# unitaryai/VTC

Measured on AMD Instinct MI355X. Metric: video-text pairs encoded/sec (config 3: 8-frame TimeSformer video + title + 5 comments, CAM) + 10k x 10k sim+R@K ms, higher is better.
Workload: dtype bf16 (video tower) + f16 (text tower blocks), fp32 accumulate; 1 GPU; configs/pretrained_clip_timesformer_comments_attention.jsonc PretrainedCLIP_TimeSformer_finaltf forward: 1024 pairs/GPU/step = 1024 videos (8 x 3 x 224 x 224) + 1024 titles + 5120 comments (77 tokens) + CAM + sim; pairs_per_gpu=1024, frames=8, text_tower=ragged: tokens after EOT are not computed, identical outputs, parallelism=dp1 (one process per GPU, no collective in the encode path)

## Files before the change

### vtc_amd/csrc/gemm.hip

```cpp
#include "gemm_common.h"
#include "ln_row.h"

#if defined(VTC_ABLATE_STORES) || defined(VTC_ABLATE_DMA) || defined(VTC_ABLATE_HALF_DMA) || defined(VTC_ABLATE_DMA_EXEC1) || \
    defined(VTC_ABLATE_VMWAIT) || defined(VTC_ABLATE_LDSREAD) || defined(VTC_PROBE_MFMA32) || defined(VTC_PHASED_WAIT_FIRST) || \
    defined(VTC_PHASED_ONE_BARRIER) || defined(VTC_NO_RELAXED_FIRST) || defined(VTC_ROW_PANEL_PROBE)
#error "timing-probe macros are not part of the product source any more (see the note above)"
#endif
#include "gemm_stamps.h"

using namespace vtcgemm;

namespace {

constexpr int MFMA_PRIO = 3;
constexpr int SMALL_NSTAGE = 3;

template <int CTRL>
__device__ __forceinline__ float dpp_f(float x) {
  return __int_as_float(__builtin_amdgcn_update_dpp(0, __float_as_int(x), CTRL, 0xf, 0xf, false));
}

template <bool NT>
__device__ __forceinline__ void store16(void *o, uint4 v) {
  typedef unsigned v4u_t __attribute__((ext_vector_type(4)));
// ... 97 lines not shown
        unsigned bits;
        if constexpr (NPL != 4) bits = __float_as_uint(acc[i][j][e]);
        else bits = (unsigned)max(__float_as_int((rn - 2.0f * acc[i][j][e]) + cn[j][e]), 0);
        constexpr unsigned KMASK = NPL != 4 ? 0x8000007Fu : 127u;
        unsigned kr = key_bfi(KMASK, (unsigned)(16 * j + 4 * g + e), bits), kc = key_bfi(KMASK, (unsigned)(16 * i + l15), bits);
        if constexpr (!INTERIOR) {
          const bool v = mv && ((cvalid >> (4 * j + e)) & 1);
          kr = v ? kr : VTC_L2MIN_INF;
          kc = v ? kc : VTC_L2MIN_INF;
        }
        row.insert(kr);
        if (cols_too) col[j][e].insert(kc);
      }
  };
#pragma unroll
  for (int i = 0; i < TM; ++i) {
    const int m = mbase + 16 * i + l15;
    const bool mv = m < p.M;
    MinR row;
    row.init();
    if (interior) row_pass(i, std::true_type{}, row);
    else row_pass(i, std::false_type{}, row);
    {
      const bool odd = (g & 1) != 0, up = g >= 2;
      unsigned o[NPLR];
#pragma unroll
      for (int q = 0; q < NPLR; ++q) o[q] = xor16_of(row.v[q], odd);
      row.merge(o);
#pragma unroll
      for (int q = 0; q < NPLR; ++q) o[q] = xor32_of(row.v[q], up);
      row.merge(o);
    }
    if (mv && nbase < p.N && g < NPLR) {
      unsigned mine = row.v[0];
#pragma unroll
      for (int q = 1; q < NPLR; ++q) mine = g == q ? row.v[q] : mine;
      p.epi.rowk[(size_t)g * rstride + (size_t)cblk * p.M + m] = mine;
    }
  }
  if (cols_too) {
    const size_t cstride = (size_t)p.epi.nblk_r * p.N;
    const int rblk = mbase / (TM * 16);
#define VTC_DPPU(x, ctrl) (unsigned)__builtin_amdgcn_update_dpp(0, (int)(x), ctrl, 0xf, 0xf, false)
    auto xor4 = [](unsigned x) -> unsigned {
      int r = __builtin_amdgcn_update_dpp(0, (int)x, 0x104, 0xf, 0x5, false);
      r = __builtin_amdgcn_update_dpp(r, (int)x, 0x114, 0xf, 0xA, false);
      return (unsigned)r;
    };
    auto step = [&](const Min4 &lo, const Min4 &hi, bool up, auto fetch) __attribute__((always_inline)) -> Min4 {
      Min4 k;
      unsigned got[NPL];
#pragma unroll
      for (int q = 0; q < NPL; ++q) {
        k.v[q] = up ? hi.v[q] : lo.v[q];
        got[q] = fetch(up ? lo.v[q] : hi.v[q]);
      }
      k.merge(got);
      return k;
    };
    const bool b0 = (l15 & 1) != 0, b1 = (l15 & 2) != 0, b2 = (l15 & 4) != 0, b3 = (l15 & 8) != 0;
    Min4 s8[8], s4[4], s2[2];
#pragma unroll
    for (int c = 0; c < 8; ++c)
      s8[c] = step(col[c >> 2][c & 3], col[(c + 8) >> 2][c & 3], b0, [](unsigned x) { return VTC_DPPU(x, 0xB1); });
#pragma unroll
    for (int c = 0; c < 4; ++c) s4[c] = step(s8[c], s8[c + 4], b1, [](unsigned x) { return VTC_DPPU(x, 0x4E); });
#pragma unroll
    for (int c = 0; c < 2; ++c) s2[c] = step(s4[c], s4[c + 2], b3, [](unsigned x) { return VTC_DPPU(x, 0x128); });
    const Min4 fin = step(s2[0], s2[1], b2, xor4);
#undef VTC_DPPU
    const int cj = (b0 ? 2 : 0) + (b1 ? 1 : 0), ce = (b3 ? 2 : 0) + (b2 ? 1 : 0);
    const int n = nbase + 16 * cj + 4 * g + ce;
    if (n < p.N && mbase < p.M) {
      unsigned *dst = p.epi.colk + (size_t)rblk * p.N + n;
#pragma unroll
      for (int q = 0; q < NPL; ++q) dst[q * cstride] = fin.v[q];
    }
  }
}

template <typename OutT, int TM>
constexpr int fast_epilogue_trailing_stores() { return TM * (sizeof(OutT) == 2 ? 2 : 4); }

template <typename T, int MODE_T, typename OutT, int WM, int WN, int TM, int TN, int SCRATCH_PER_WAVE, bool REJOIN = false>
__device__ __forceinline__ void tile_epilogue(f32x4 (&acc)[TM][TN], const GemmParams &p, int m0, int n0, unsigned scratch_off) {
  constexpr bool FOLD = MODE_T >= EPI_FOLD_BASE && MODE_T <= EPI_RESID_FOLD_C;
  constexpr bool CENTER = MODE_T == EPI_RESID_FOLD_C;
  constexpr int MODE = CENTER ? VTC_EPI_RESID : (FOLD ? MODE_T - EPI_FOLD_BASE : MODE_T);
  auto rejoin = [&]() __attribute__((always_inline)) {
    if constexpr (REJOIN) {
      if ((int)(threadIdx.x >> 6) / WN == 0) __builtin_amdgcn_s_barrier();
    }
  };
  if constexpr (MODE == EPI_L2MIN || l2min_half_keys(MODE)) {
    rejoin();
    if constexpr (TN == 4) l2min_epilogue<WM, WN, TM, TN, l2min_row_planes(MODE), l2min_col_planes(MODE)>(acc, p, m0, n0);
    return;
  }
  extern __shared__ __attribute__((aligned(16))) char lds[];
  constexpr int BM = WM * TM * 16, BN = WN * TN * 16;
  int tid = threadIdx.x;
  asm volatile("" : "+v"(tid));
  const int lane = tid & 63, wave = tid >> 6;
  const int wr = wave / WN, wc = wave % WN;
  const int g = lane >> 4;
  const int ldo = p.ldo;
  const bool vec_ok = (ldo & 3) == 0;
  constexpr bool nt_out = MODE == EPI_L2DIST || (sizeof(OutT) == 2 && MODE != VTC_EPI_RESID && MODE != EPI_RESID_LN);
  const bool interior = (m0 + BM <= p.M) && (n0 + BN <= p.N) && vec_ok;
  float scale = 1.0f;
  if (MODE == EPI_SCALE) scale = __expf(*p.epi.scale_log);
  if constexpr (sizeof(OutT) == 2) {
    if (interior) {
      constexpr int TSB = 136;
      char *trb = lds + scratch_off + wave * SCRATCH_PER_WAVE;
      const int l15 = lane & 15;
      const int ncol0 = n0 + wc * TN * 16;
      float4 b4[TN];
      if (p.bias) {
#pragma unroll
        for (int j = 0; j < TN; ++j) b4[j] = *reinterpret_cast<const float4 *>(p.bias + ncol0 + 16 * j + 4 * g);
      } else {
#pragma unroll
        for (int j = 0; j < TN; ++j) b4[j] = make_float4(0.f, 0.f, 0.f, 0.f);
      }
      [[maybe_unused]] float *fold_rs = reinterpret_cast<float *>(trb + 2 * 16 * TSB);
      [[maybe_unused]] float *fold_sc = fold_rs + 2 * TM * 16;
      constexpr int NQ = (TM * 16 + 63) / 64;
      [[maybe_unused]] float2 fst[NQ];
      [[maybe_unused]] float4 fsc = make_float4(0.f, 0.f, 0.f, 0.f);
      if constexpr (FOLD) {
        static_assert(2 * 16 * TSB + (2 * TM * 16 + TN * 16) * 4 <= SCRATCH_PER_WAVE, "folded LayerNorm: row statistics + s in the wave's scratch");
#pragma unroll
        for (int q = 0; q < NQ; ++q) {
          const int r = min(lane + 64 * q, TM * 16 - 1);
          fst[q] = *reinterpret_cast<const float2 *>(p.epi.fold_stat + 2 * (size_t)(m0 + wr * TM * 16 + r));
        }
        fsc = *reinterpret_cast<const float4 *>(p.epi.fold_s + ncol0 + 4 * (lane & (TN * 4 - 1)));
      }
      rejoin();
      if constexpr (FOLD) {
#pragma unroll
        for (int q = 0; q < NQ; ++q) {
          const int r = lane + 64 * q;
          if (TM * 16 % 64 == 0 || r < TM * 16) *reinterpret_cast<float2 *>(fold_rs + 2 * r) = fst[q];
        }
        if (lane < TN * 4) *reinterpret_cast<float4 *>(fold_sc + 4 * lane) = fsc;
        __builtin_amdgcn_fence(__ATOMIC_RELEASE, "wavefront");
        __builtin_amdgcn_wave_barrier();
        __builtin_amdgcn_fence(__ATOMIC_ACQUIRE, "wavefront");
      }
      auto put = [&](int i) __attribute__((always_inline)) {
        char *buf = trb + (i & 1) * (16 * TSB);
#pragma unroll
        for (int j = 0; j < TN; ++j) {
          float v0, v1, v2, v3;
          if constexpr (FOLD) {
            const float2 st = *reinterpret_cast<const float2 *>(fold_rs + 2 * (i * 16 + l15));
            const float4 sj = *reinterpret_cast<const float4 *>(fold_sc + 16 * j + 4 * g);
            typedef float f2_t __attribute__((ext_vector_type(2)));
            const f2_t nmu = {-st.x, -st.x}, rs = {st.y, st.y};
            const f2_t t01 = __builtin_elementwise_fma(nmu, (f2_t){sj.x, sj.y}, (f2_t){acc[i][j][0], acc[i][j][1]});
            const f2_t t23 = __builtin_elementwise_fma(nmu, (f2_t){sj.z, sj.w}, (f2_t){acc[i][j][2], acc[i][j][3]});
            const f2_t w01 = __builtin_elementwise_fma(rs, t01, (f2_t){b4[j].x, b4[j].y});
            const f2_t w23 = __builtin_elementwise_fma(rs, t23, (f2_t){b4[j].z, b4[j].w});
            v0 = w01.x; v1 = w01.y; v2 = w23.x; v3 = w23.y;
          } else {
            v0 = acc[i][j][0] + b4[j].x; v1 = acc[i][j][1] + b4[j].y; v2 = acc[i][j][2] + b4[j].z; v3 = acc[i][j][3] + b4[j].w;
          }
          if (MODE == VTC_EPI_GELU) {
            if constexpr (sizeof(T) == 4) {
              v0 = quick_gelu<true>(v0); v1 = quick_gelu<true>(v1); v2 = quick_gelu<true>(v2); v3 = quick_gelu<true>(v3);
            } else {
              const gelu_f2_t g01 = quick_gelu2((gelu_f2_t){v0, v1}), g23 = quick_gelu2((gelu_f2_t){v2, v3});
              v0 = g01.x; v1 = g01.y; v2 = g23.x; v3 = g23.y;
            }
          }
          uint2 pk;
          pk.x = pack16<OutT>(v0, v1);
          pk.y = pack16<OutT>(v2, v3);
          *reinterpret_cast<uint2 *>(buf + l15 * TSB + j * 32 + g * 8) = pk;
        }
      };
      static_assert(2 * 16 * TSB <= SCRATCH_PER_WAVE, "two transposition buffers per wave");
      static_assert(fast_epilogue_trailing_stores<OutT, TM>() == TM * 2, "16-bit fast path: TM fragment rows x 2 stores (the loop below)");
      char *out_base16;
      {
        const int m0s = __builtin_amdgcn_readfirstlane(m0), wrs = __builtin_amdgcn_readfirstlane(wr), ncs = __builtin_amdgcn_readfirstlane(ncol0);
        out_base16 = reinterpret_cast<char *>(reinterpret_cast<unsigned short *>(p.out) + (size_t)(m0s + wrs * TM * 16) * ldo + ncs);
      }
      put(0);
#pragma unroll
      for (int i = 0; i < TM; ++i) {
        __builtin_amdgcn_fence(__ATOMIC_RELEASE, "wavefront");
        __builtin_amdgcn_wave_barrier();
        __builtin_amdgcn_fence(__ATOMIC_ACQUIRE, "wavefront");
        const char *buf = trb + (i & 1) * (16 * TSB);
        uint2 lo[2], hi[2];
#pragma unroll
        for (int k = 0; k < 2; ++k) {
          const int r = (lane >> 3) + 8 * k, c = lane & 7;
          lo[k] = *reinterpret_cast<const uint2 *>(buf + r * TSB + c * 16);
          hi[k] = *reinterpret_cast<const uint2 *>(buf + r * TSB + c * 16 + 8);
        }
        if (i + 1 < TM) put(i + 1);
#pragma unroll
        for (int k = 0; k < 2; ++k) {
          char *o = out_base16 + (unsigned)(((i * 16 + (lane >> 3) + 8 * k) * ldo + (lane & 7) * 8) * 2);
          store16<nt_out>(o, make_uint4(lo[k].x, lo[k].y, hi[k].x, hi[k].y));
        }
      }
      __builtin_amdgcn_fence(__ATOMIC_RELEASE, "wavefront");
      __builtin_amdgcn_wave_barrier();
      return;
    }
  }
  [[maybe_unused]] __amdgpu_buffer_rsrc_t out_rsrc;
  [[maybe_unused]] const int m0u = __builtin_amdgcn_readfirstlane(m0);
  if constexpr (MODE == EPI_RESID_LN || MODE == VTC_EPI_RESID) {
    const size_t rem = (size_t)(p.M - m0u) * ldo * 4;
    out_rsrc = __builtin_amdgcn_make_buffer_rsrc(reinterpret_cast<float *>(p.out) + (size_t)m0u * ldo, 0,
                                                 (int)(rem < 0xFFFFFFF0u ? rem : 0xFFFFFFF0u), 0x00020000);
  }
  if (sizeof(OutT) == 4 && interior) {
    constexpr int TS = 68;
    constexpr int H = TN / 4, NP = TM * H;
    static_assert(TN % 4 == 0 && (H == 1 || sizeof(OutT) == 4), "wide wave tiles: fp32 outputs only");
    static_assert(sizeof(OutT) == 2 || fast_epilogue_trailing_stores<OutT, TM>() <= NP * 4, "fp32 fast path: NP passes x 4 stores (>= the count the K loop's relaxed waits assume)");
    float *tr = reinterpret_cast<float *>(lds + scratch_off + wave * SCRATCH_PER_WAVE);
    const int l15 = lane & 15;
    const int ncol0 = n0 + wc * TN * 16;
    const float *colv = MODE == EPI_L2DIST ? p.epi.coln : p.bias;
    float cadd[H][8];
#pragma unroll
    for (int hh = 0; hh < H; ++hh)
#pragma unroll
      for (int e = 0; e < 8; ++e) cadd[hh][e] = 0.f;
    if (colv) {
#pragma unroll
      for (int hh = 0; hh < H; ++hh) {
        const float4 c4 = *reinterpret_cast<const float4 *>(colv + ncol0 + 64 * hh + l15 * 4);
        cadd[hh][0] = c4.x; cadd[hh][1] = c4.y; cadd[hh][2] = c4.z; cadd[hh][3] = c4.w;
      }
    }
    auto fin = [&](float a, float add) -> float {
      float v = a + add;
      if (MODE == VTC_EPI_GELU) v = quick_gelu<sizeof(T) == 4>(v);
      if (MODE == EPI_SCALE) v *= scale;
      return v;
    };
    auto x_ptr = [&](int pp, int k) -> float * {
      const int m = m0 + (wr * TM + pp / H) * 16 + (lane >> 4) + 4 * k;
      return reinterpret_cast<float *>(p.out) + (size_t)m * ldo + ncol0 + 64 * (pp % H) + l15 * 4;
    };
    constexpr int XD = 2;
    float4 xr[XD][4];
    constexpr bool SPLIT = FOLD && MODE == VTC_EPI_RESID && sizeof(T) == 2;
    [[maybe_unused]] float *mean_prev = tr + 16 * TS;
    [[maybe_unused]] float2 *stat_buf = reinterpret_cast<float2 *>(tr + 16 * TS + TM * 16);
    constexpr int NQM = (TM * 16 + 63) / 64;
    [[maybe_unused]] float mprev[NQM];
    if constexpr (SPLIT && CENTER) {
      static_assert((16 * TS + TM * 16) * 4 <= SCRATCH_PER_WAVE, "folded LayerNorm: previous means in the wave's scratch");
#pragma unroll
      for (int q = 0; q < NQM; ++q) mprev[q] = p.epi.fold_stat[2 * (size_t)(m0 + wr * TM * 16 + min(lane + 64 * q, TM * 16 - 1))];
    }
    typedef unsigned v2u_t __attribute__((ext_vector_type(2)));
    [[maybe_unused]] char *hi_base = nullptr, *lo_base = nullptr;
    [[maybe_unused]] unsigned split_off0 = 0, split_row4 = 0;
    if constexpr (SPLIT) {
      const int m0s = __builtin_amdgcn_readfirstlane(m0);
      const int wrs = __builtin_amdgcn_readfirstlane(wr), ncs = __builtin_amdgcn_readfirstlane(ncol0);
      const size_t row0 = (size_t)(m0s + wrs * TM * 16) * ldo + ncs;
      hi_base = reinterpret_cast<char *>(reinterpret_cast<unsigned short *>(p.epi.y16) + row0);
      lo_base = reinterpret_cast<char *>(reinterpret_cast<unsigned short *>(p.epi.y16lo) + row0);
      split_off0 = (unsigned)(((lane >> 4) * ldo + l15 * 4) * 2);
      split_row4 = (unsigned)ldo * 8u;
    }
    auto split_off = [&](int pp, int k) -> unsigned { return split_off0 + (unsigned)(4 * (pp / H) + k) * split_row4 + (unsigned)(128 * (pp % H)); };
    auto x_load = [&](int pp, int k) -> float4 {
      if constexpr (SPLIT) {
        const v2u_t hi = *reinterpret_cast<const v2u_t *>(hi_base + split_off(pp, k));
        const v2u_t lo = *reinterpret_cast<const v2u_t *>(lo_base + split_off(pp, k));
        return make_float4(__uint_as_float(hi.x), __uint_as_float(hi.y), __uint_as_float(lo.x), __uint_as_float(lo.y));
      } else {
        return *reinterpret_cast<const float4 *>(x_ptr(pp, k));
      }
    };
    [[maybe_unused]] unsigned skip_rem = 1, skip_step = 0, skip_m = 0;
    if constexpr (MODE == VTC_EPI_RESID || MODE == EPI_RESID_LN) {
      if (p.epi.skip_mod > 0) {
        skip_m = (unsigned)p.epi.skip_mod;
// ... 265 lines not shown
      const unsigned w_addr = lds_base + cur * STAGE + A_BYTES + wrow;
#pragma unroll
      for (int ks = 0; ks < 2; ++ks) {
        if (ks == 1 && late_dma) issued = stage_ahead(t, NSTAGE - 1);
        const unsigned coff = ((4 * ks + g) ^ swz) << 4;
        u32x4 wf[TN], aE, aO;
#pragma unroll
        for (int j = 0; j < TN; ++j) lds_read16(wf[j], w_addr + coff, j * 16 * ROWB);
        lds_read16(aE, a_addr + coff, 0);
#pragma unroll
        for (int i = 0; i < TM; i += 2) {
          lds_read16(aO, a_addr + coff, (i + 1) * 16 * ROWB);
          if (i == 0) lgkm_wait_frags<1>(aE, wf);
          else lgkm_wait<1>(aE);
#pragma unroll
          for (int j = 0; j < TN; ++j) Mma<T>::run(wf[j], aE, acc[i][j]);
          if (i + 2 < TM) {
            lds_read16(aE, a_addr + coff, (i + 2) * 16 * ROWB);
            lgkm_wait<1>(aO);
          } else {
            lgkm_wait<0>(aO);
          }
#pragma unroll
          for (int j = 0; j < TN; ++j) Mma<T>::run(wf[j], aO, acc[i + 1][j]);
        }
      }
      if (issued) ++ahead;
      wait_all_but(ahead - 1);
      --ahead;
      __syncthreads();
      cur = cur + 1 == NSTAGE ? 0 : cur + 1;
    }

    tile_epilogue<T, MODE, OutT, WM, WN, TM, TN, STAGE / NW>(acc, p, m0, n0, ((cur + NSTAGE - 1) % NSTAGE) * STAGE);
    if (has_next) __syncthreads();

    if (!has_next) break;
    li += nb_x; m0 = m0n; n0 = n0n;
    tile_offsets<AG>(a_off, m0, p.M, p.lda_bytes, wave_u, lane);
    tile_offsets<WG>(w_off, n0, p.N, p.ldw_bytes, wave_u, lane);
    has_next = li + nb_x < nt_x;
    if (has_next) decode(start_x + li + nb_x, m0n, n0n);
  }
}


template <typename T16>
__device__ __attribute__((noinline)) void fused_ln_rows(const float *out, int M, int N, int m0, const float *ln_g, const float *ln_b,
                                                        T16 *ln_out) {
  typedef unsigned v4u_t __attribute__((ext_vector_type(4)));
  const __amdgpu_buffer_rsrc_t x_rsrc = __builtin_amdgcn_make_buffer_rsrc(const_cast<float *>(out), 0, (int)((size_t)M * N * 4), 0x00020000);
  const int lane = threadIdx.x & 63, wave = threadIdx.x >> 6;
  const int width = N;
  const int rows = min(256, M - m0);
  constexpr int RB = 8;
  for (int r0 = wave; r0 < rows; r0 += 8 * RB) {
    float4 v[RB][LN_MAXV][2];
#pragma unroll
    for (int b = 0; b < RB; ++b) {
      const int r = min(r0 + 8 * b, rows - 1);
#pragma unroll
      for (int i = 0; i < LN_MAXV; ++i) {
        const int c = min((lane + 64 * i) * 8, width - 8);
        const int off = (int)(((size_t)(m0 + r) * width + c) * 4);
        const v4u_t a = __builtin_amdgcn_raw_buffer_load_b128(x_rsrc, off, 0, 16);
        const v4u_t b4 = __builtin_amdgcn_raw_buffer_load_b128(x_rsrc, off + 16, 0, 16);
        v[b][i][0] = make_float4(__uint_as_float(a.x), __uint_as_float(a.y), __uint_as_float(a.z), __uint_as_float(a.w));
        v[b][i][1] = make_float4(__uint_as_float(b4.x), __uint_as_float(b4.y), __uint_as_float(b4.z), __uint_as_float(b4.w));
      }
    }
#pragma unroll
    for (int b = 0; b < RB; ++b) {
      const int r = r0 + 8 * b;
      if (r < rows) ln_row_compute<T16, false>(v[b], ln_g, ln_b, ln_out + (size_t)(m0 + r) * width, width, lane);
    }
  }
}

template <int MODE, typename OutT, typename T, int DEEP = 0>
__global__ __launch_bounds__(512, 2) void gemm_phased_kernel(GemmParams p) {
  static_assert(sizeof(T) == 2, "16-bit operands (bf16 or IEEE half)");
  static_assert(DEEP == 0 || DEEP == 1, "0 = one quarter in flight, 1 = deep (W0 re-read)");
  constexpr int WM = 2, WN = 4, TM = 8, TN = 4, NW = 8, BM = 256, BN = 256;
  if (p.epi.m_dev) {
    p.M = *p.epi.m_dev;
    p.MT = (p.M + BM - 1) / BM;
  }
  constexpr int A_BYTES = BM * ROWB, STAGE = (BM + BN) * ROWB;
  extern __shared__ __attribute__((aligned(16))) char lds[];
  const int tid = threadIdx.x, lane = tid & 63, wave = tid >> 6;
  const int wr = wave >> 2, wc = wave & 3;
  const int g = lane >> 4;

  [[maybe_unused]] const int bid = blockIdx.x;
  const XcdRange rng = xcd_range(p.MT * p.NT);
  const int nb_x = rng.nb_x, nt_x = rng.nt_x, start_x = rng.start_x;
  auto decode = [&](int logical, int &m0, int &n0) { decode_tile<BM, BN>(logical, 1, p.MT, p.NT, m0, n0); };
  int li = rng.slot;
  if (li >= nt_x) return;
  int m0, n0;
  decode(start_x + li, m0, n0);
  int m0n = 0, n0n = 0;
  bool has_next = li + nb_x < nt_x;
  if (has_next) decode(start_x + li + nb_x, m0n, n0n);

  const int ksteps = p.K / 64;
  const unsigned lds_base = __builtin_amdgcn_readfirstlane((unsigned)(size_t)(lds_void *)lds);
  const int wave_u = __builtin_amdgcn_readfirstlane(wave);
  const int swz = (lane >> 1) & 7;
  const unsigned a_rd = (wr * 128 + (lane & 15)) * ROWB;
  const unsigned w_rd = A_BYTES + (wc * 64 + (lane & 15)) * ROWB;
  const unsigned coff0 = ((0 + g) ^ swz) << 4, coff1 = ((4 + g) ^ swz) << 4;
  unsigned ra0 = lds_base + a_rd + coff0, ra1 = lds_base + a_rd + coff1, rw0 = lds_base + w_rd + coff0, rw1 = lds_base + w_rd + coff1;
  int rd_step = STAGE;

  const int ga0 = (wave_u >> 2) * 16 + (wave_u & 3) * 2;
  const int gw0 = (wave_u >> 1) * 8 + (wave_u & 1) * 2;
  const unsigned a_vo = (unsigned)(lane >> 3) * (unsigned)p.lda_bytes + (((lane & 7) ^ (lane >> 4)) << 4);
  const unsigned w_vo = (unsigned)(lane >> 3) * (unsigned)p.ldw_bytes + (((lane & 7) ^ (lane >> 4)) << 4);
  const unsigned a_vo2 = (a_vo ^ 64u) + 8u * (unsigned)p.lda_bytes - 1024u, w_vo2 = (w_vo ^ 64u) + 8u * (unsigned)p.ldw_bytes - 1024u;
  const unsigned offA0 = (unsigned)ga0 * 8u * (unsigned)p.lda_bytes, offA1 = (unsigned)(ga0 + 8) * 8u * (unsigned)p.lda_bytes;
  const unsigned offW0 = (unsigned)gw0 * 8u * (unsigned)p.ldw_bytes, offW1 = (unsigned)(gw0 + 4) * 8u * (unsigned)p.ldw_bytes;
  const char *tbA = p.A + (size_t)m0 * p.lda_bytes, *tbW = p.W + (size_t)n0 * p.ldw_bytes;
  const char *tbAn = p.A + (size_t)m0n * p.lda_bytes, *tbWn = p.W + (size_t)n0n * p.ldw_bytes;
  auto stage2 = [&](const char *base, const char *tile_base, unsigned grp_off, int row0, int nrows, int ld_bytes, unsigned vo, unsigned vo2, int grp,
                    int kb, unsigned lds_dst, bool fast) __attribute__((always_inline)) {
    if (__builtin_expect(fast, 1)) {
      const char *sb0 = tile_base + (grp_off + (unsigned)kb);
      asm volatile(
          "s_mov_b32 m0, %3\n\t"
          "s_nop 0\n\t"
          "global_load_lds_dwordx4 %0, %2\n\t"
          "global_load_lds_dwordx4 %1, %2 offset:1024"
          :
          : "v"(vo), "v"(vo2), "s"(sb0), "s"(lds_dst)
          : "memory");
    } else {
#pragma unroll
      for (int q = 0; q < 2; ++q) {
        const int r = (grp + q) * 8 + (lane >> 3);
        const int c = (lane & 7) ^ ((r >> 1) & 7);
        int gr = row0 + r;
        gr = gr < nrows ? gr : nrows - 1;
        glds16(base + (size_t)gr * ld_bytes + kb + c * 16, __builtin_amdgcn_readfirstlane(lds_dst + q * 1024));
      }
    }
  };
  constexpr bool CAN_GATHER = MODE == EPI_PATCH && sizeof(T) == 2;
  const bool gather = CAN_GATHER && p.epi.gather;
  [[maybe_unused]] unsigned gvo[4] = {0, 0, 0, 0};
  [[maybe_unused]] const int g_cs = p.epi.patch == 32 ? 2 : 1;
  auto gather_offsets = [&](int sm) __attribute__((always_inline)) {
    if constexpr (CAN_GATHER) {
      const int P = p.epi.P, G = p.epi.grid, res = p.epi.res, ps = p.epi.patch;
#pragma unroll
      for (int h = 0; h < 2; ++h)
#pragma unroll
        for (int q = 0; q < 2; ++q) {
          const int m = min(sm + (ga0 + 8 * h + q) * 8 + (lane >> 3), p.M - 1);
          const int f = m / P, np = m - f * P;
          const int gy = np / G, gx = np - gy * G;
          const int c = ((lane & 7) ^ (lane >> 4)) ^ (q << 2);
          const unsigned origin = (unsigned)(((f * 3) * res + gy * ps) * res + gx * ps) * 2u;
          gvo[2 * h + q] = origin + (unsigned)((c >> g_cs) * res * 2 + ((c & ((1 << g_cs) - 1)) << 4));
        }
    }
  };
  auto gather_kbase = [&](int kk) -> size_t {
    const int k = kk * 64, pp = p.epi.patch * p.epi.patch;
    const int c = k / pp, i = (k - c * pp) / p.epi.patch;
    return ((size_t)c * p.epi.res + i) * p.epi.res * 2;
  };
  enum { Q_A0 = 0, Q_W0 = 1, Q_W1 = 2, Q_A1 = 3 };
  auto stage_quarter = [&](int qi, int sm, int sn, int kk, unsigned st, bool fastA, bool fastW, const char *ta, const char *tw) __attribute__((always_inline)) {
    if (qi == Q_A0 || qi == Q_A1) {
      const int grp = ga0 + (qi == Q_A1 ? 8 : 0);
      if constexpr (CAN_GATHER) {
        if (gather) {
          const char *sb0 = reinterpret_cast<const char *>(p.A) + gather_kbase(kk);
          const char *sb1 = sb0 - 1024;
          const int h = qi == Q_A1 ? 1 : 0;
          asm volatile(
              "s_mov_b32 m0, %4\n\t"
              "s_nop 0\n\t"
              "global_load_lds_dwordx4 %0, %2\n\t"
              "global_load_lds_dwordx4 %1, %3 offset:1024"
              :
              : "v"(gvo[2 * h]), "v"(gvo[2 * h + 1]), "s"(sb0), "s"(sb1), "s"(st + grp * 1024)
              : "memory");
          return;
        }
      }
      stage2(p.A, ta, qi == Q_A1 ? offA1 : offA0, sm, p.M, p.lda_bytes, a_vo, a_vo2, grp, kk * ROWB, st + grp * 1024, fastA);
    } else {
      const int grp = gw0 + (qi == Q_W1 ? 4 : 0);
      stage2(p.W, tw, qi == Q_W1 ? offW1 : offW0, sn, p.N, p.ldw_bytes, w_vo, w_vo2, grp, kk * ROWB, st + A_BYTES + grp * 1024, fastW);
    }
  };

  int cur = 0;
  {
    const bool fa = m0 + BM <= p.M, fw = n0 + BN <= p.N;
    if (gather) gather_offsets(m0);
#pragma unroll
    for (int qi = 0; qi < 4; ++qi) stage_quarter(qi, m0, n0, 0, lds_base, fa, fw, tbA, tbW);
    asm volatile("s_waitcnt vmcnt(0)" ::: "memory");
    __builtin_amdgcn_s_barrier();
  }

  u32x4 aS[4][2], wS[2][2];
  bool relax_first = false;
  [[maybe_unused]] float *nrm = reinterpret_cast<float *>(lds + 2 * STAGE);
  [[maybe_unused]] auto fetch_norm = [&](int tm0, int tn0) -> float {
    if (tid < 256) {
      const int m = tm0 + tid;
      return m < p.M ? -0.5f * p.epi.rown[m] : 0.f;
    }
    const int n = tn0 + tid - 256;
    return n < p.N ? -0.5f * p.epi.coln[n] : 0.f;
  };
  if constexpr (l2min_half_keys(MODE)) {
    nrm[tid] = fetch_norm(m0, n0);
    __syncthreads();
  }
  VTC_STAMP_INIT();
  while (true) {
    if (wr == 1) __builtin_amdgcn_s_barrier();
    f32x4 acc[TM][TN];
#pragma unroll
    for (int i = 0; i < TM; ++i)
#pragma unroll
      for (int j = 0; j < TN; ++j) {
        if constexpr (l2min_half_keys(MODE)) {
          const float hr = nrm[wr * 128 + 16 * i + (lane & 15)];
          const float4 hc = *reinterpret_cast<const float4 *>(nrm + 256 + wc * 64 + 16 * j + 4 * g);
          acc[i][j] = (f32x4){hr + hc.x, hr + hc.y, hr + hc.z, hr + hc.w};
        } else {
          acc[i][j] = (f32x4){0.f, 0.f, 0.f, 0.f};
        }
      }

    auto kloop = [&](auto all_fast_c) __attribute__((always_inline)) {
    constexpr bool ALL_FAST = decltype(all_fast_c)::value;
    for (int t = 0; t < ksteps; ++t) {
      const unsigned st_cur = lds_base + cur * STAGE, st_nxt = lds_base + (cur ^ 1) * STAGE;
      if constexpr (DEEP == 0) {
        const int kn = t + 1;
        const bool to_next = kn == ksteps && has_next;
        const int sm = to_next ? m0n : m0, sn = to_next ? n0n : n0, kk = kn < ksteps ? kn : 0;
        const bool fastA = ALL_FAST || sm + BM <= p.M, fastW = ALL_FAST || sn + BN <= p.N;
        const char *ta = to_next ? tbAn : tbA, *tw = to_next ? tbWn : tbW;
        if constexpr (CAN_GATHER) {
          if (gather && to_next) gather_offsets(m0n);
        }
        static_for<4>([&](auto ph_c) __attribute__((always_inline)) {
          constexpr int ph = decltype(ph_c)::value;
          constexpr int qm = ph >> 1, qn = (ph == 1 || ph == 2) ? 1 : 0;
          if constexpr (ph != 2) {
  #pragma unroll
            for (int j = 0; j < 2; ++j) {
              lds_read16(wS[j][0], rw0, (qn * 2 + j) * 16 * ROWB);
              lds_read16(wS[j][1], rw1, (qn * 2 + j) * 16 * ROWB);
            }
          }
          if constexpr (ph == 0 || ph == 2) {
  #pragma unroll
            for (int i = 0; i < 4; ++i) {
              lds_read16(aS[i][0], ra0, (qm * 4 + i) * 16 * ROWB);
              lds_read16(aS[i][1], ra1, (qm * 4 + i) * 16 * ROWB);
            }
          }
          stage_quarter(ph, sm, sn, kk, st_nxt, fastA, fastW, ta, tw);
          __builtin_amdgcn_s_barrier();
          lgkm_wait_subtile(aS, wS);
          __builtin_amdgcn_s_setprio(MFMA_PRIO);
  #pragma unroll
          for (int ks = 0; ks < 2; ++ks)
  #pragma unroll
            for (int i = 0; i < 4; ++i)
  #pragma unroll
              for (int j = 0; j < 2; ++j) Mma<T>::run(wS[j][ks], aS[i][ks], acc[qm * 4 + i][qn * 2 + j]);
          __builtin_amdgcn_s_setprio(0);
          constexpr int NST = fast_epilogue_trailing_stores<OutT, TM>();
          if (ph < 2 && t == 0 && relax_first) {
            if constexpr (ph == 0) asm volatile("s_waitcnt vmcnt(%0)" ::"n"(2 + NST) : "memory");
            else asm volatile("s_waitcnt vmcnt(%0)" ::"n"(4 + NST) : "memory");
          } else
            asm volatile("s_waitcnt vmcnt(2)" ::: "memory");
          __builtin_amdgcn_s_barrier();
        });
      } else {
        constexpr int NST = fast_epilogue_trailing_stores<OutT, TM>();
        const bool first = t == 0, last = t == ksteps - 1;
        const bool nx1 = t + 1 == ksteps && has_next;
        const int sm1 = nx1 ? m0n : m0, sn1 = nx1 ? n0n : n0, kk1 = t + 1 < ksteps ? t + 1 : 0;
        const bool fA1 = ALL_FAST || sm1 + BM <= p.M, fW1 = ALL_FAST || sn1 + BN <= p.N;
        const char *ta1 = nx1 ? tbAn : tbA, *tw1 = nx1 ? tbWn : tbW;
        const bool nx2 = t + 2 >= ksteps && has_next;
        const int sm2 = nx2 ? m0n : m0, sn2 = nx2 ? n0n : n0, kk2 = t + 2 < ksteps ? t + 2 : 0;
        const bool fA2 = ALL_FAST || sm2 + BM <= p.M, fW2 = ALL_FAST || sn2 + BN <= p.N;
        const char *ta2 = nx2 ? tbAn : tbA, *tw2 = nx2 ? tbWn : tbW;
        static_for<4>([&](auto ph_c) __attribute__((always_inline)) {
          constexpr int ph = decltype(ph_c)::value;
          constexpr int qm = ph >> 1, qn = (ph == 1 || ph == 2) ? 1 : 0;
          if constexpr (ph == 0 || ph == 1 || ph == 3) {
#pragma unroll
            for (int j = 0; j < 2; ++j) {
              lds_read16(wS[j][0], rw0, (qn * 2 + j) * 16 * ROWB);
              lds_read16(wS[j][1], rw1, (qn * 2 + j) * 16 * ROWB);
            }
          }
          if constexpr (ph == 0 || ph == 2) {
#pragma unroll
            for (int i = 0; i < 4; ++i) {
              lds_read16(aS[i][0], ra0, (qm * 4 + i) * 16 * ROWB);
              lds_read16(aS[i][1], ra1, (qm * 4 + i) * 16 * ROWB);
            }
          }
          if constexpr (ph == 0) {
            stage_quarter(Q_W0, sm1, sn1, kk1, st_nxt, fA1, fW1, ta1, tw1);
            if (first) stage_quarter(Q_A0, sm1, sn1, kk1, st_nxt, fA1, fW1, ta1, tw1);
          } else if constexpr (ph == 1) {
            if (first) stage_quarter(Q_W1, sm1, sn1, kk1, st_nxt, fA1, fW1, ta1, tw1);
            stage_quarter(Q_A1, sm1, sn1, kk1, st_nxt, fA1, fW1, ta1, tw1);
            if (first && relax_first) asm volatile("s_waitcnt vmcnt(%0)" ::"n"(8 + NST) : "memory");
            else asm volatile("s_waitcnt vmcnt(8)" ::: "memory");
          } else if constexpr (ph == 2) {
            if (!last) {
              if constexpr (CAN_GATHER) {
                if (gather && nx2 && t + 2 == ksteps) gather_offsets(m0n);
              }
              stage_quarter(Q_A0, sm2, sn2, kk2, st_cur, fA2, fW2, ta2, tw2);
            }
          } else {
            if (!last) stage_quarter(Q_W1, sm2, sn2, kk2, st_cur, fA2, fW2, ta2, tw2);
            lgkm_wait_w4(wS);
            if (last) asm volatile("s_waitcnt vmcnt(2)" ::: "memory");
            else asm volatile("s_waitcnt vmcnt(6)" ::: "memory");
          }
          __builtin_amdgcn_s_barrier();
          lgkm_wait_subtile(aS, wS);
          VTC_PHASE_STAMP(1);
          __builtin_amdgcn_s_setprio(MFMA_PRIO);
#pragma unroll
          for (int ks = 0; ks < 2; ++ks)
#pragma unroll
            for (int i = 0; i < 4; ++i)
#pragma unroll
              for (int j = 0; j < 2; ++j) Mma<T>::run(wS[j][ks], aS[i][ks], acc[qm * 4 + i][qn * 2 + j]);
          __builtin_amdgcn_s_setprio(0);
          VTC_PHASE_STAMP(0);
          __builtin_amdgcn_s_barrier();
        });
      }
      cur ^= 1;
      ra0 += rd_step; ra1 += rd_step; rw0 += rd_step; rw1 += rd_step;
      rd_step = -rd_step;
    }
    };
    if constexpr (MODE != EPI_L2MIN && !l2min_half_keys(MODE) && MODE != EPI_PATCH && MODE != EPI_RESID_LN) {
      const bool this_in = m0 + BM <= p.M && n0 + BN <= p.N, next_in = !has_next || (m0n + BM <= p.M && n0n + BN <= p.N);
      if (this_in && next_in) kloop(std::true_type{});
      else kloop(std::false_type{});
    } else {
      kloop(std::false_type{});
    }
    VTC_STAMP(0);
    VTC_STAMP(1);

    [[maybe_unused]] float nrm_next = 0.f;
    if constexpr (l2min_half_keys(MODE)) {
      if (has_next) nrm_next = fetch_norm(m0n, n0n);
    }
    tile_epilogue<T, MODE, OutT, WM, WN, TM, TN, STAGE / NW, true>(acc, p, m0, n0, (cur ^ 1) * STAGE);
    if constexpr (MODE == EPI_RESID_LN) {
      int *ticket = reinterpret_cast<int *>(lds + 2 * STAGE);
      asm volatile("s_waitcnt vmcnt(0)" ::: "memory");
      __syncthreads();
      if (tid == 0) *ticket = __hip_atomic_fetch_add(p.epi.ln_cnt + m0 / BM, 1, __ATOMIC_RELAXED, __HIP_MEMORY_SCOPE_AGENT);
      __syncthreads();
      if (*ticket == p.NT - 1)
        fused_ln_rows<T>(reinterpret_cast<const float *>(p.out), p.M, p.N, m0, p.epi.ln_g, p.epi.ln_b, reinterpret_cast<T *>(p.epi.ln_out));
    }
    VTC_STAMP_TILE_END(!has_next);
    if (!has_next) break;
    relax_first = MODE != EPI_L2MIN && !l2min_half_keys(MODE) && MODE != EPI_RESID_LN && (m0 + BM <= p.M) && (n0 + BN <= p.N) && ((p.ldo & 3) == 0);
    if constexpr (l2min_half_keys(MODE)) {
      nrm[tid] = nrm_next;
      asm volatile("s_waitcnt lgkmcnt(0)" ::: "memory");
    }
    __builtin_amdgcn_s_barrier();
    VTC_STAMP(3);
    li += nb_x; m0 = m0n; n0 = n0n;
    tbA = tbAn; tbW = tbWn;
    has_next = li + nb_x < nt_x;
    if (has_next) {
      decode(start_x + li + nb_x, m0n, n0n);
      tbAn = p.A + (size_t)m0n * p.lda_bytes; tbWn = p.W + (size_t)n0n * p.ldw_bytes;
    }
  }
}


}
namespace vtcgemm {
int num_cus() {
  static std::atomic<int> cus[64];
  int dev = 0;
  if (hipGetDevice(&dev) != hipSuccess || dev < 0 || dev >= 64) dev = 0;
  int n = cus[dev].load(std::memory_order_relaxed);
  if (n == 0) {
    int v = 0;
    if (hipDeviceGetAttribute(&v, hipDeviceAttributeMultiprocessorCount, dev) != hipSuccess || v <= 0) v = 256;
    cus[dev].store(n = v, std::memory_order_relaxed);
  }
  return n;
}
}
namespace {

template <typename T, int MODE, typename OutT, int WM, int WN, int TM, int TN, int NSTAGE>
int run(GemmParams p, hipStream_t stream) {
  constexpr int BM = WM * TM * 16, BN = WN * TN * 16, NT_ = WM * WN * 64;
  p.MT = cdiv(p.M, BM); p.NT = cdiv(p.N, BN);
  const int S = p.epi.ksplit > 1 ? p.epi.ksplit : 1;
  const int ntiles = p.MT * p.NT * S;
  const size_t shmem = (size_t)NSTAGE * (BM + BN) * ROWB;
  if (p.K / S / Mma<T>::KPR < NSTAGE - 1) { vtc_set_error("gemm: K=%d (/ %d slices) is too short for %d stages", p.K, S, NSTAGE); return 1; }
  const int wg_per_cu = shmem > 80 * 1024 ? 1 : 2;
  const int grid = min(ntiles, num_cus() * wg_per_cu);
  if (S > 1 && (grid < ntiles || p.K % (S * Mma<T>::KPR) != 0)) {
    vtc_set_error("gemm: split-K x %d needs one workgroup per (tile, slice) (%d > %d resident) and K %% (slices x %d) == 0 (K=%d)", S, ntiles, grid, Mma<T>::KPR, p.K);
    return 1;
  }
  static PerDeviceOnce attr;
  if (ensure_dynamic_lds(attr, reinterpret_cast<const void *>(&gemm_kernel<T, MODE, OutT, WM, WN, TM, TN, NSTAGE>), (int)shmem, "gemm")) return 1;
  hipLaunchKernelGGL((gemm_kernel<T, MODE, OutT, WM, WN, TM, TN, NSTAGE>), dim3(grid), dim3(NT_), shmem, stream, p);
  VTC_LAUNCH_CHECK("gemm");
  return 0;
}

template <int MODE, typename OutT, typename T, int DEEP>
int run_phased_d(GemmParams p, hipStream_t stream) {
  p.MT = cdiv(p.M, 256); p.NT = cdiv(p.N, 256);
  const int ntiles = p.MT * p.NT;
  const size_t shmem = (size_t)2 * 512 * ROWB + (MODE == EPI_RESID_LN ? 16 : 0) + (l2min_half_keys(MODE) ? 2048 : 0);
  const int grid = min(ntiles, num_cus());
  static PerDeviceOnce attr;
  if (ensure_dynamic_lds(attr, reinterpret_cast<const void *>(&gemm_phased_kernel<MODE, OutT, T, DEEP>), (int)shmem, "gemm_phased")) return 1;
  VTC_STAMP_HOST_BEFORE(p, stream);
  hipLaunchKernelGGL((gemm_phased_kernel<MODE, OutT, T, DEEP>), dim3(grid), dim3(512), shmem, stream, p);
  VTC_STAMP_HOST_AFTER(p, stream, grid, MODE);
  VTC_LAUNCH_CHECK("gemm_phased");
  return 0;
}
template <int MODE, typename OutT, typename T>
int run_phased(const GemmParams &p, hipStream_t stream) {
  if constexpr (MODE != EPI_RESID_LN && MODE != EPI_L2MIN && !l2min_half_keys(MODE)) {
    if (p.K >= 128) return run_phased_d<MODE, OutT, T, 1>(p, stream);
  }
  return run_phased_d<MODE, OutT, T, 0>(p, stream);
}

enum class Tile { Phased256, Small128, Small64 };
struct TileChoice {
  Tile tile;
  int nstage;
};
constexpr TileChoice choose_tile(int M, int N, int K, int elem_bytes, int ksplit, int cus) {
  const int ksteps = K / (ksplit > 1 ? ksplit : 1) / (ROWB / elem_bytes);
  const TileChoice small64 = {Tile::Small64, ksteps >= SMALL_NSTAGE - 1 ? SMALL_NSTAGE : 2};
  if (ksplit > 1) return small64;
  if (elem_bytes == 2) {
    const long tb = (long)cdiv(M, 256) * cdiv(N, 256), ts = (long)cdiv(M, 128) * cdiv(N, 128);
    const long rb = (tb + cus - 1) / cus, rs = (ts + 2 * cus - 1) / (2 * cus);
    if (rb * 100 <= rs * 65) return {Tile::Phased256, 2};
  }
  const long ts128 = (long)cdiv(M, 128) * cdiv(N, 128);
  if (ts128 * 2 <= cus) return small64;
  return {Tile::Small128, 2};
}
constexpr Tile tile_at_256_cus(int M, int N, int elem_bytes = 2) { return choose_tile(M, N, 768, elem_bytes, 0, 256).tile; }
static_assert(tile_at_256_cus(12800, 768) == Tile::Phased256, "150 big tiles: big");
static_assert(tile_at_256_cus(25344, 768) == Tile::Small128, "297 big tiles: small");
static_assert(tile_at_256_cus(6400, 768) == Tile::Small128, "75 big tiles: small");
static_assert(tile_at_256_cus(32768, 512) == Tile::Phased256, "256 big tiles: big");
static_assert(tile_at_256_cus(38400, 768) == Tile::Phased256, "450 big tiles: big");
static_assert(tile_at_256_cus(12800, 768, 4) != Tile::Phased256 && tile_at_256_cus(32768, 512, 4) != Tile::Phased256, "fp32 operands: never the phased kernel");
static_assert(tile_at_256_cus(1024, 2048) == Tile::Small64 && tile_at_256_cus(1024 + 128, 2048) == Tile::Small128, "64 x 64 while tiles128 * 2 <= cus");
static_assert(choose_tile(128, 128, 64, 2, 0, 256).nstage == 2 && choose_tile(128, 128, 128, 2, 0, 256).nstage == SMALL_NSTAGE &&
                  choose_tile(128, 128, 192, 2, 0, 256).nstage == SMALL_NSTAGE && choose_tile(128, 128, 256, 2, 4, 256).nstage == 2,
              "64 x 64 stages: 2 for one K-step (of a slice), 3 from two K-steps on");

template <typename T, int MODE, typename OutT>
int run_cfg(const GemmParams &p, hipStream_t stream) {
  const TileChoice c = choose_tile(p.M, p.N, p.K, sizeof(T), p.epi.ksplit, num_cus());
  if constexpr (sizeof(T) == 2) {
    if (c.tile == Tile::Phased256) return run_phased<MODE, OutT, T>(p, stream);
  }
  if (c.tile == Tile::Small64) {
    if (c.nstage == SMALL_NSTAGE) return run<T, MODE, OutT, 2, 1, 2, 4, SMALL_NSTAGE>(p, stream);
    return run<T, MODE, OutT, 2, 1, 2, 4, 2>(p, stream);
  }
  return run<T, MODE, OutT, 2, 2, 4, 4, 2>(p, stream);
}

int run_l2min(const GemmParams &p, hipStream_t stream) {
  if (p.epi.mode == EPI_L2MIN2) return run_phased<EPI_L2MIN2, float, bf16_t>(p, stream);
  if (p.epi.mode == EPI_L2MIN3) return run_phased<EPI_L2MIN3, float, bf16_t>(p, stream);
  return run_phased<EPI_L2MIN, float, bf16_t>(p, stream);
}

template <typename T>
int dispatch(GemmParams p, hipStream_t stream) {
  const bool out_f32 = p.epi.out_dtype == VTC_F32;
  using Out16 = std::conditional_t<sizeof(T) == 2, T, bf16_t>;
  switch (p.epi.mode) {
    case VTC_EPI_STORE:
      if (out_f32) return run_cfg<T, VTC_EPI_STORE, float>(p, stream);
      if constexpr (sizeof(T) == 2) {
        if (p.epi.fold_stat) return run_cfg<T, EPI_STORE_FOLD, Out16>(p, stream);
      }
      return run_cfg<T, VTC_EPI_STORE, Out16>(p, stream);
    case VTC_EPI_GELU:
      if (out_f32) return run_cfg<T, VTC_EPI_GELU, float>(p, stream);
      if constexpr (sizeof(T) == 2) {
        if (p.epi.fold_stat) return run_cfg<T, EPI_GELU_FOLD, Out16>(p, stream);
      }
      return run_cfg<T, VTC_EPI_GELU, Out16>(p, stream);
// ... 106 lines not shown
```

Before: 8967 pairs/s.

## Park last epilogue rows and drip their stores into next tile's first k-step

For the deep phased GEMM with 16-bit store/GELU outputs, the epilogue now holds back its last four fragment rows (one in a dedicated LDS buffer, three in registers) instead of storing them immediately. Those rows are then written out during the four phases of the next tile's first k-step, interleaved with the MFMA work, so the epilogue's store tail overlaps with compute. This adds LDS, register pressure, extra tile lookahead decoding (two tiles ahead), and adjusted vmcnt waits, and it only applies when this tile and the next two are fully interior.

```diff
diff --git a/vtc_amd/csrc/gemm.hip b/vtc_amd/csrc/gemm.hip
--- a/vtc_amd/csrc/gemm.hip
+++ b/vtc_amd/csrc/gemm.hip
@@ -203,8 +203,23 @@
 template <typename OutT, int TM>
 constexpr int fast_epilogue_trailing_stores() { return TM * (sizeof(OutT) == 2 ? 2 : 4); }
 
-template <typename T, int MODE_T, typename OutT, int WM, int WN, int TM, int TN, int SCRATCH_PER_WAVE, bool REJOIN = false>
-__device__ __forceinline__ void tile_epilogue(f32x4 (&acc)[TM][TN], const GemmParams &p, int m0, int n0, unsigned scratch_off) {
+template <int TN, int ROWS>
+struct ParkedRows {
+  static constexpr int TSB = 136;
+  static constexpr int LDS_OFF = 2 * 512 * ROWB;
+  static constexpr int LDS_BYTES = 8 * 16 * TSB;
+  uint2 w[ROWS > 1 ? ROWS - 1 : 1][TN];
+  char *base;
+  unsigned voff, rstep;
+};
+template <int MODE, typename OutT, int DEEP>
+constexpr int park_rows() {
+  return DEEP == 1 && sizeof(OutT) == 2 && (MODE == VTC_EPI_STORE || MODE == VTC_EPI_GELU || MODE == EPI_STORE_FOLD || MODE == EPI_GELU_FOLD) ? 4 : 0;
+}
+
+template <typename T, int MODE_T, typename OutT, int WM, int WN, int TM, int TN, int SCRATCH_PER_WAVE, bool REJOIN = false, int PARK = 0>
+__device__ __forceinline__ void tile_epilogue(f32x4 (&acc)[TM][TN], const GemmParams &p, int m0, int n0, unsigned scratch_off,
+                                              [[maybe_unused]] bool park = false, [[maybe_unused]] ParkedRows<TN, PARK> *parked = nullptr) {
   constexpr bool FOLD = MODE_T >= EPI_FOLD_BASE && MODE_T <= EPI_RESID_FOLD_C;
   constexpr bool CENTER = MODE_T == EPI_RESID_FOLD_C;
   constexpr int MODE = CENTER ? VTC_EPI_RESID : (FOLD ? MODE_T - EPI_FOLD_BASE : MODE_T);
@@ -313,6 +328,9 @@
       put(0);
 #pragma unroll
       for (int i = 0; i < TM; ++i) {
+        if constexpr (PARK > 0) {
+          if (park && i >= TM - PARK) break;
+        }
         __builtin_amdgcn_fence(__ATOMIC_RELEASE, "wavefront");
         __builtin_amdgcn_wave_barrier();
         __builtin_amdgcn_fence(__ATOMIC_ACQUIRE, "wavefront");
@@ -324,11 +342,36 @@
           lo[k] = *reinterpret_cast<const uint2 *>(buf + r * TSB + c * 16);
           hi[k] = *reinterpret_cast<const uint2 *>(buf + r * TSB + c * 16 + 8);
         }
-        if (i + 1 < TM) put(i + 1);
+        if constexpr (PARK > 0) {
+          if (i + 1 < TM && !(park && i + 1 >= TM - PARK)) put(i + 1);
+        } else {
+          if (i + 1 < TM) put(i + 1);
+        }
 #pragma unroll
         for (int k = 0; k < 2; ++k) {
           char *o = out_base16 + (unsigned)(((i * 16 + (lane >> 3) + 8 * k) * ldo + (lane & 7) * 8) * 2);
           store16<nt_out>(o, make_uint4(lo[k].x, lo[k].y, hi[k].x, hi[k].y));
+        }
+      }
+      if constexpr (PARK > 0) {
+        static_assert(nt_out && PARK < TM && ParkedRows<TN, PARK>::TSB == TSB, "parked rows: the 16-bit store / QuickGELU modes");
+        if (park) {
+          char *db = lds + ParkedRows<TN, PARK>::LDS_OFF + wave * (16 * TSB);
+#pragma unroll
+          for (int r = 0; r < PARK; ++r) {
+            const int i = TM - PARK + r;
+            put(i);
+            const char *buf = trb + (i & 1) * (16 * TSB);
+#pragma unroll
+            for (int j = 0; j < TN; ++j) {
+              const uint2 own = *reinterpret_cast<const uint2 *>(buf + l15 * TSB + j * 32 + g * 8);
+              if (r == 0) *reinterpret_cast<uint2 *>(db + l15 * TSB + j * 32 + g * 8) = own;
+              else parked->w[r - 1][j] = own;
+            }
+          }
+          parked->base = out_base16;
+          parked->voff = (unsigned)((((TM - PARK) * 16 + (lane >> 3)) * ldo + (lane & 7) * 8) * 2);
+          parked->rstep = (unsigned)__builtin_amdgcn_readfirstlane(ldo) * 16u;
         }
       }
       __builtin_amdgcn_fence(__ATOMIC_RELEASE, "wavefront");
@@ -760,6 +803,7 @@
   static_assert(sizeof(T) == 2, "16-bit operands (bf16 or IEEE half)");
   static_assert(DEEP == 0 || DEEP == 1, "0 = one quarter in flight, 1 = deep (W0 re-read)");
   constexpr int WM = 2, WN = 4, TM = 8, TN = 4, NW = 8, BM = 256, BN = 256;
+  constexpr int PARK = park_rows<MODE, OutT, DEEP>();
   if (p.epi.m_dev) {
     p.M = *p.epi.m_dev;
     p.MT = (p.M + BM - 1) / BM;
@@ -814,6 +858,18 @@
           : "v"(vo), "v"(vo2), "s"(sb0), "s"(lds_dst)
           : "memory");
     } else {
+      if constexpr (PARK > 0) {
+        int ln = lane;
+        asm volatile("" : "+v"(ln));
+#pragma unroll
+        for (int q = 0; q < 2; ++q) {
+          const int r = (grp + q) * 8 + (ln >> 3);
+          const int c = (ln & 7) ^ ((r >> 1) & 7);
+          int gr = row0 + r;
+          gr = gr < nrows ? gr : nrows - 1;
+          glds16(base + (size_t)gr * ld_bytes + kb + c * 16, __builtin_amdgcn_readfirstlane(lds_dst + q * 1024));
+        }
+      } else {
 #pragma unroll
       for (int q = 0; q < 2; ++q) {
         const int r = (grp + q) * 8 + (lane >> 3);
@@ -821,6 +877,7 @@
         int gr = row0 + r;
         gr = gr < nrows ? gr : nrows - 1;
         glds16(base + (size_t)gr * ld_bytes + kb + c * 16, __builtin_amdgcn_readfirstlane(lds_dst + q * 1024));
+      }
       }
     }
   };
@@ -888,6 +945,9 @@
 
   u32x4 aS[4][2], wS[2][2];
   bool relax_first = false;
+  [[maybe_unused]] ParkedRows<TN, PARK> parked;
+  [[maybe_unused]] bool drip = false;
+  [[maybe_unused]] int t_first = 0;
   [[maybe_unused]] float *nrm = reinterpret_cast<float *>(lds + 2 * STAGE);
   [[maybe_unused]] auto fetch_norm = [&](int tm0, int tn0) -> float {
     if (tid < 256) {
@@ -918,9 +978,10 @@
         }
       }
 
-    auto kloop = [&](auto all_fast_c) __attribute__((always_inline)) {
+    auto kloop = [&](auto all_fast_c, auto drip_c) __attribute__((always_inline)) {
     constexpr bool ALL_FAST = decltype(all_fast_c)::value;
-    for (int t = 0; t < ksteps; ++t) {
+    constexpr bool DRIP = decltype(drip_c)::value;
+    for (int t = (PARK > 0 && !DRIP ? t_first : 0); t < (DRIP ? 1 : ksteps); ++t) {
       const unsigned st_cur = lds_base + cur * STAGE, st_nxt = lds_base + (cur ^ 1) * STAGE;
       if constexpr (DEEP == 0) {
         const int kn = t + 1;
@@ -969,7 +1030,16 @@
         });
       } else {
         constexpr int NST = fast_epilogue_trailing_stores<OutT, TM>();
-        const bool first = t == 0, last = t == ksteps - 1;
+        const bool first = DRIP || t == 0, last = !DRIP && t == ksteps - 1;
+        [[maybe_unused]] char *db_wr = nullptr;
+        [[maybe_unused]] const char *db_rd = nullptr;
+        if constexpr (DRIP) {
+          int dt = threadIdx.x;
+          asm volatile("" : "+v"(dt));
+          char *db = lds + ParkedRows<TN, PARK>::LDS_OFF + (dt >> 6) * (16 * ParkedRows<TN, PARK>::TSB);
+          db_wr = db + (dt & 15) * ParkedRows<TN, PARK>::TSB + ((dt & 63) >> 4) * 8;
+          db_rd = db + ((dt & 63) >> 3) * ParkedRows<TN, PARK>::TSB + (dt & 7) * 16;
+        }
         const bool nx1 = t + 1 == ksteps && has_next;
         const int sm1 = nx1 ? m0n : m0, sn1 = nx1 ? n0n : n0, kk1 = t + 1 < ksteps ? t + 1 : 0;
         const bool fA1 = ALL_FAST || sm1 + BM <= p.M, fW1 = ALL_FAST || sn1 + BN <= p.N;
@@ -981,6 +1051,21 @@
         static_for<4>([&](auto ph_c) __attribute__((always_inline)) {
           constexpr int ph = decltype(ph_c)::value;
           constexpr int qm = ph >> 1, qn = (ph == 1 || ph == 2) ? 1 : 0;
+          [[maybe_unused]] uint2 dlo[2], dhi[2];
+          if constexpr (DRIP && ph < PARK) {
+            __builtin_amdgcn_fence(__ATOMIC_RELEASE, "wavefront");
+            __builtin_amdgcn_wave_barrier();
+            __builtin_amdgcn_fence(__ATOMIC_ACQUIRE, "wavefront");
+#pragma unroll
+            for (int k = 0; k < 2; ++k) {
+              dlo[k] = *reinterpret_cast<const uint2 *>(db_rd + 8 * k * ParkedRows<TN, PARK>::TSB);
+              dhi[k] = *reinterpret_cast<const uint2 *>(db_rd + 8 * k * ParkedRows<TN, PARK>::TSB + 8);
+            }
+            if constexpr (ph + 1 < PARK) {
+#pragma unroll
+              for (int j = 0; j < TN; ++j) *reinterpret_cast<uint2 *>(db_wr + j * 32) = parked.w[ph][j];
+            }
+          }
           if constexpr (ph == 0 || ph == 1 || ph == 3) {
 #pragma unroll
             for (int j = 0; j < 2; ++j) {
@@ -1001,7 +1086,8 @@
           } else if constexpr (ph == 1) {
             if (first) stage_quarter(Q_W1, sm1, sn1, kk1, st_nxt, fA1, fW1, ta1, tw1);
             stage_quarter(Q_A1, sm1, sn1, kk1, st_nxt, fA1, fW1, ta1, tw1);
-            if (first && relax_first) asm volatile("s_waitcnt vmcnt(%0)" ::"n"(8 + NST) : "memory");
+            if constexpr (DRIP) asm volatile("s_waitcnt vmcnt(%0)" ::"n"(8 + (TM - PARK) * 2 + 2) : "memory");
+            else if (first && relax_first) asm volatile("s_waitcnt vmcnt(%0)" ::"n"(8 + NST) : "memory");
             else asm volatile("s_waitcnt vmcnt(8)" ::: "memory");
           } else if constexpr (ph == 2) {
             if (!last) {
@@ -1013,12 +1099,18 @@
           } else {
             if (!last) stage_quarter(Q_W1, sm2, sn2, kk2, st_cur, fA2, fW2, ta2, tw2);
             lgkm_wait_w4(wS);
-            if (last) asm volatile("s_waitcnt vmcnt(2)" ::: "memory");
+            if constexpr (DRIP) asm volatile("s_waitcnt vmcnt(%0)" ::"n"(6 + 4) : "memory");
+            else if (last) asm volatile("s_waitcnt vmcnt(2)" ::: "memory");
             else asm volatile("s_waitcnt vmcnt(6)" ::: "memory");
           }
           __builtin_amdgcn_s_barrier();
           lgkm_wait_subtile(aS, wS);
           VTC_PHASE_STAMP(1);
+          if constexpr (DRIP && ph < PARK) {
+#pragma unroll
+            for (int k = 0; k < 2; ++k)
+              store16<true>(parked.base + (parked.voff + (unsigned)(2 * ph + k) * parked.rstep), make_uint4(dlo[k].x, dlo[k].y, dhi[k].x, dhi[k].y));
+          }
           __builtin_amdgcn_s_setprio(MFMA_PRIO);
 #pragma unroll
           for (int ks = 0; ks < 2; ++ks)
@@ -1038,10 +1130,21 @@
     };
     if constexpr (MODE != EPI_L2MIN && !l2min_half_keys(MODE) && MODE != EPI_PATCH && MODE != EPI_RESID_LN) {
       const bool this_in = m0 + BM <= p.M && n0 + BN <= p.N, next_in = !has_next || (m0n + BM <= p.M && n0n + BN <= p.N);
-      if (this_in && next_in) kloop(std::true_type{});
-      else kloop(std::false_type{});
+      if (this_in && next_in) {
+        if constexpr (PARK > 0) {
+          t_first = 0;
+          if (drip) {
+            kloop(std::true_type{}, std::true_type{});
+            t_first = 1;
+          }
+        }
+        kloop(std::true_type{}, std::false_type{});
+      } else {
+        if constexpr (PARK > 0) t_first = 0;
+        kloop(std::false_type{}, std::false_type{});
+      }
     } else {
-      kloop(std::false_type{});
+      kloop(std::false_type{}, std::false_type{});
     }
     VTC_STAMP(0);
     VTC_STAMP(1);
@@ -1050,7 +1153,18 @@
     if constexpr (l2min_half_keys(MODE)) {
       if (has_next) nrm_next = fetch_norm(m0n, n0n);
     }
-    tile_epilogue<T, MODE, OutT, WM, WN, TM, TN, STAGE / NW, true>(acc, p, m0, n0, (cur ^ 1) * STAGE);
+    [[maybe_unused]] bool park = false, has_nn = false;
+    [[maybe_unused]] int m0nn = 0, n0nn = 0;
+    if constexpr (PARK > 0) {
+      if (has_next) {
+        has_nn = li + 2 * nb_x < nt_x;
+        if (has_nn) decode(start_x + li + 2 * nb_x, m0nn, n0nn);
+        park = (m0 + BM <= p.M) && (n0 + BN <= p.N) && (m0n + BM <= p.M) && (n0n + BN <= p.N) && (!has_nn || ((m0nn + BM <= p.M) && (n0nn + BN <= p.N))) &&
+               ((p.ldo & 3) == 0);
+      }
+    }
+    if constexpr (PARK > 0) tile_epilogue<T, MODE, OutT, WM, WN, TM, TN, STAGE / NW, true, PARK>(acc, p, m0, n0, (cur ^ 1) * STAGE, park, &parked);
+    else tile_epilogue<T, MODE, OutT, WM, WN, TM, TN, STAGE / NW, true>(acc, p, m0, n0, (cur ^ 1) * STAGE);
     if constexpr (MODE == EPI_RESID_LN) {
       int *ticket = reinterpret_cast<int *>(lds + 2 * STAGE);
       asm volatile("s_waitcnt vmcnt(0)" ::: "memory");
@@ -1071,10 +1185,19 @@
     VTC_STAMP(3);
     li += nb_x; m0 = m0n; n0 = n0n;
     tbA = tbAn; tbW = tbWn;
-    has_next = li + nb_x < nt_x;
-    if (has_next) {
-      decode(start_x + li + nb_x, m0n, n0n);
-      tbAn = p.A + (size_t)m0n * p.lda_bytes; tbWn = p.W + (size_t)n0n * p.ldw_bytes;
+    if constexpr (PARK > 0) {
+      drip = park;
+      has_next = has_nn;
+      if (has_next) {
+        m0n = m0nn; n0n = n0nn;
+        tbAn = p.A + (size_t)m0n * p.lda_bytes; tbWn = p.W + (size_t)n0n * p.ldw_bytes;
+      }
+    } else {
+      has_next = li + nb_x < nt_x;
+      if (has_next) {
+        decode(start_x + li + nb_x, m0n, n0n);
+        tbAn = p.A + (size_t)m0n * p.lda_bytes; tbWn = p.W + (size_t)n0n * p.ldw_bytes;
+      }
     }
   }
 }
@@ -1122,7 +1245,8 @@
 int run_phased_d(GemmParams p, hipStream_t stream) {
   p.MT = cdiv(p.M, 256); p.NT = cdiv(p.N, 256);
   const int ntiles = p.MT * p.NT;
-  const size_t shmem = (size_t)2 * 512 * ROWB + (MODE == EPI_RESID_LN ? 16 : 0) + (l2min_half_keys(MODE) ? 2048 : 0);
+  const size_t shmem = (size_t)2 * 512 * ROWB + (MODE == EPI_RESID_LN ? 16 : 0) + (l2min_half_keys(MODE) ? 2048 : 0) +
+                       (park_rows<MODE, OutT, DEEP>() > 0 ? ParkedRows<4, 4>::LDS_BYTES : 0);
   const int grid = min(ntiles, num_cus());
   static PerDeviceOnce attr;
   if (ensure_dynamic_lds(attr, reinterpret_cast<const void *>(&gemm_phased_kernel<MODE, OutT, T, DEEP>), (int)shmem, "gemm_phased")) return 1;
```

Result: slower. 8776 pairs/s (-2.1%).
